# kai0511/insider

Measured on AMD Instinct MI355X. Metric: outer-iterations/sec (masked INSIDER fit, 10000 x 50000, K=30), higher is better.
Workload: dtype f64

## Files before the change

### insider_amd/csrc/insider_hip.hip

```cpp
#include "insider_kernels.hpp"
#include "insider_posthoc.hpp"
#include "insider_vardecomp.hpp"
#include "insider_sampdecomp.hpp"
#include "insider_levelscores.hpp"
#include "insider_factdecomp.hpp"
#include "insider_rescomp.hpp"
#include "insider_outliers.hpp"
#include "insider_neighbors.hpp"
#include "insider_enrich.hpp"
#include "insider_kmeans.hpp"
#include "insider_tsne.hpp"

#include <rccl/rccl.h>

#include <algorithm>
#include <chrono>
#include <cstdlib>
#include <cmath>
#include <cstdio>
#include <cstring>
#include <limits>
#include <memory>
#include <mutex>
#include <atomic>
// ... 227 lines not shown
};

struct Workspace {
    static constexpr int EARLY = 3;
    int K = 0, NB = 0, KP = 0, nseg = 1;
    int gram_blocks_p = 0, gram_blocks_n = 0, sc_blocks = 0;
    DevBuf<double> Astack, R, C, RtR, CCt, Qfull, SC, stat, stat_col, gram_part, sc_part, lvl_part, eq, lvl_sum;
    DevBuf<double> fperm;
    DevBuf<double> lvl_zero;
    DevBuf<double> Qheld;
    DevBuf<double> U, Ylvl, wpart, Vlev;
    DevBuf<double> lvl_sum_all;
    DevBuf<double> gram_part2, sc_part2;
    DevBuf<double> wg_part;
    DevBuf<uint8_t> wg_pair;
    DevBuf<double> sse_train, sse_test, b2, b1, loss_buf, stage;
    size_t stage_count = 0;
    DevBuf<int> sweeps, failflag;
    DevBuf<int> sweep_key;
    DevBuf<unsigned long long> sweep_total;
    DevBuf<unsigned> pc4_ticket;
    unsigned pc4_base[2] = {0, 0};
    unsigned long long cd_code_base = 0, cd_pair_base = 0;
    DevBuf<unsigned long long> code_base_dev;
    uint8_t *order = nullptr;
    DevBuf<uint8_t> order_buf[2];
    int order_rows = 0;
    DevBuf<int> gene_perm;
    DevBuf<int> sched_cnt[2], sched_rank;
    DevBuf<uint16_t> sched_bkt;
    int sched_flip = 0;
    DevBuf<double> cd_hsave, cd_isave;
    DevBuf<uint32_t> cd_pass_slot;
    DevBuf<int> cd_pass_perm[2], cd_pass_cnt;
    DevBuf<int> perm_early[EARLY];
    bool have_early[EARLY] = {false, false, false};
    bool have_perm = false;
};

constexpr unsigned EV_SYNC = hipEventDisableTiming | hipEventDisableSystemFence;

struct Join {
    Event ev;
    bool pending = false;
    int record(hipStream_t s) { HIPCHECK(hipEventRecord(ev, s)); pending = true; return INSIDER_OK; }
    int wait(hipStream_t s)
    {
        if (pending) HIPCHECK(hipStreamWaitEvent(s, ev, 0));
        pending = false;
        return INSIDER_OK;
    }
    void drop() { pending = false; }
};

struct Streams {
    Stream stream;
    Stream side;
    Stream side2;
    Stream side3;
    Event ev_cd_done, ev_prep, ev_c_ready;
    Event ev_head;
    std::vector<Event> ev_w;
    Event ev_a_ready, ev_tab;
    Join qfull, qheld, side_done;

    int create(int n_w)
    {
        HIPCHECK(hipStreamCreate(stream.out()));
        for (Stream *s : {&side, &side2, &side3}) HIPCHECK(hipStreamCreateWithFlags(s->out(), hipStreamNonBlocking));
        for (Event *e : {&ev_prep, &ev_c_ready, &ev_head, &ev_a_ready, &qfull.ev, &qheld.ev, &ev_cd_done, &side_done.ev, &ev_tab})
            HIPCHECK(hipEventCreateWithFlags(e->out(), EV_SYNC));
        ev_w.resize(n_w);
        for (Event &e : ev_w) HIPCHECK(hipEventCreateWithFlags(e.out(), EV_SYNC));
        return INSIDER_OK;
    }
    int synchronize_sides() const
    {
        for (const Stream *s : {&side, &side2, &side3}) HIPCHECK(hipStreamSynchronize(*s));
        return INSIDER_OK;
    }
    void synchronize() const
    {
        for (const Stream *s : {&stream, &side, &side2, &side3}) if (*s) (void)hipStreamSynchronize(*s);
    }
};

struct Options {
    int max_sweeps = 1 << 24, order_mode = 0, profile = 0, verbose = 0, cd_variant = 0, force_allreduce = 0;
    int col_factored = 1;
    int row_counts = 1;
    int row_merged = 1;
    int row_gemm = 1;
    int wg_waves = 1024;
    int row_fused = 1;
    int mm_fast = 1;
    int mm_tiles = 0;
    int col_mfma4 = 1;
    int cd_pairs = 1;
    int list_fine = 1;
    int cd_cold_iters = 3, cd_pass_first = 64, cd_pass_ratio = 4;
    double resid_stage_mb = 256.0;
    double vd_stage_kb = 48.0;
    int sd_slabs = 0;
    int ls_slabs = 0;
    double ls_part_mb = 256.0;
    int glm_slabs = 0;
    int rc_slabs = 0;
};

struct PostWs {
    DevBuf<double> Ast, U, cp, part, stats, stage, gpart, gram, cpart, gsum, L, dinv, outs;
    DevBuf<int> nz, ints, info;
    DevBuf<double> vin, vtab, vrec;
    DevBuf<double> spart, srec;
    DevBuf<double> lcand, ltab, lpart, lcnt, lout;
    DevBuf<double> fwall, fprod, fbase, frec;
    DevBuf<double> rq, rcs, rz, rpart, rin, rout;
    DevBuf<double> ocs, oz;
    DevBuf<uint32_t> obits;
    DevBuf<int> ogcnt, oscnt, orows, ocols;
    DevBuf<long long> ooffs;
};

}

struct insider_hip_handle {
    std::shared_ptr<const DataSet> ds;
    Streams st;
    Options opt;
    Workspace ws;
    PostWs post;
    FitPlan plan;
    bool w_ready = false;
    int64_t gene_offset = 0;
    int rank = 0, world = 1;
    insider_allreduce_fn allreduce = nullptr;
    void *allreduce_user = nullptr;
    ncclComm_t comm = nullptr;
    std::vector<Event> ev_col, ev_row, ev_cd, ev_test;
    double prof[12] = {0, 0, 0, 0, 0, 0, 0, 0, 0, 0, 0, 0};
    double steady_cd_ms = 0, steady_col_ms = 0;
    int cap_hits = 0, max_gene_sweeps = 0;
    int col_solver = 0, col_eval = 0, col_ridge_fallback = 0;
    int col_stats_kernel = 0, col_stats_tickets = 0, col_stats_blocks = 0;
    int col_q_kernel = 0, mm_rows2_tiles = 0;
    uint64_t row_kernels = 0;
    int vd_path = 0;
    int sd_path = 0, sd_slabs = 0;
    int ls_path = 0, ls_slabs = 0;
    int glm_slabs = 0, glm_form = 0;
    int fd_path = 0;
    int rc_slabs = 0;
    double rc_ms = 0.0;
    int ol_path = 0;

    ~insider_hip_handle()
    {
        if (ds) (void)hipSetDevice(ds->device);
        st.synchronize();
        if (comm) (void)ncclCommDestroy(comm);
    }
};

namespace {

constexpr int PC4_PARTS = 16;
constexpr int MM_SLAB = 128;

enum RowKernel {
    RK_WGEMM4 = 0, RK_WGEMM5, RK_WGEMM6, RK_WGEMM7, RK_WGEMM_CHUNKS, RK_WSYRK, RK_GRAM_SIDE,
    RK_GENE_U_CNT, RK_GENE_U, RK_GENE_UC,
    RK_MERGED_SOLVE, RK_MERGED, RK_MERGED_ZERO, RK_PACK_REDUCE,
    RK_LIST_STATS4, RK_LIST_STATS, RK_LEVEL_PARTIAL, RK_LEVEL_SOLVE, RK_CONT_CD,
    RK_MM_ROWS2, RK_MM_ROWS, RK_MM_REDUCE2_2, RK_MM_REDUCE2_4, RK_MM_REDUCE
};
inline uint64_t rk_bit(RowKernel k) { return 1ull << (int)k; }
inline void row_mark(insider_hip_handle *h, RowKernel k) { h->row_kernels |= rk_bit(k); }

PlanFacts plan_facts(const insider_hip_handle *h, int K)
{
    const DataSet &d = *h->ds;
    PlanFacts f;
    const Options &o = h->opt;
    f.opt = {o.row_merged, o.col_factored, o.row_fused, o.row_gemm, o.row_counts, o.mm_fast, o.force_allreduce, o.wg_waves};
    f.world = h->world;
    f.K = K; f.NB = h->ws.NB; f.KP = h->ws.KP; f.lvl_zero = (bool)h->ws.lvl_zero;
    f.merged = d.merged; f.cont_merged = d.cont_merged; f.cf_pair_ok = d.cf_pair_ok; f.cf_hn = (bool)d.cf_hn; f.cf_zt = (bool)d.cf_zt;
    f.c = d.c; f.m = d.m; f.SL = d.SL; f.SLcat = d.SLcat; f.p = d.p; f.col_entries = d.col_entries; f.row_entries = d.row_entries;
    for (const CovTables &ct : d.cov) { f.L.push_back(ct.L); f.npairs.push_back(ct.npairs); }
    f.cf_c = d.cf.c; f.cf_tab_rows = d.cf.tab_rows; f.cf_nsteps = d.cf.nsteps;
    std::copy(d.cf.L, d.cf.L + CF_MAXC + 1, f.cf_L);
    std::copy(d.cf.nlater, d.cf.nlater + CF_MAXC + 1, f.cf_nlater);
    return f;
}

int ensure_workspace(insider_hip_handle *h, int K)
{
    if (K < 1 || K > INSIDER_MAX_K) return fail(INSIDER_ERR_UNSUPPORTED, "K must be in 1..63");
    if (h->ws.K == K) return INSIDER_OK;
    h->ws = Workspace();
    const DataSet &d = *h->ds;
    const hipStream_t st = h->st.stream;
    Workspace w;
    const int NB = (K + 1 + 15) / 16, KP = 16 * NB, NBLK = NB * (NB + 1) / 2, STAT = NBLK * 256;
    w.NB = NB;
    w.KP = KP;
    const int64_t avg_batches = (int64_t)(d.row_entries / (uint64_t)LIST_ALIGN / (uint64_t)std::max<int64_t>(d.n, 1));
    int nseg = (int)std::min<int64_t>(std::max<int64_t>(1, cdiv(8192, d.n)), std::max<int64_t>(1, avg_batches / 16));
    nseg = std::min(nseg, 64);
    w.nseg = nseg;
    w.gram_blocks_p = cdiv(d.p, MM_SLAB);
    w.gram_blocks_n = cdiv(d.n, MM_SLAB);
    w.sc_blocks = cdiv(d.p, MM_SLAB);
    const size_t rec = STAT + 2 * KP + 2, max_L = std::max(d.max_L, 1);
    int rc;
    if ((rc = w.Astack.alloc((size_t)(d.SL + 16) * KP))) return rc;
    HIPCHECK(hipMemset(w.Astack, 0, (size_t)(d.SL + 16) * KP * sizeof(double)));
// ... 35 lines not shown
                }
            if ((rc = w.wg_pair.upload(ab))) return rc;
        }
        if ((rc = w.U.alloc((size_t)d.p * round_up(max_L, 2)))) return rc;
        if ((rc = w.Ylvl.alloc(max_L * KP))) return rc;
        if ((rc = w.wpart.alloc((size_t)std::max(d.max_items, 1) * STAT))) return rc;
        if ((rc = w.lvl_sum_all.alloc((size_t)std::max(d.SL, 1) * rec))) return rc;
        if ((rc = w.gram_part2.alloc((size_t)std::max(w.gram_blocks_p, w.gram_blocks_n) * KP * KP))) return rc;
        if ((rc = w.sc_part2.alloc((size_t)w.sc_blocks * d.SL * KP))) return rc;
        if ((rc = w.Vlev.alloc((size_t)d.p * d.SLP))) return rc;
        HIPCHECK(hipMemsetAsync(w.Vlev, 0, (size_t)d.p * d.SLP * sizeof(double), st));
        if ((rc = w.Qheld.alloc((size_t)d.p * KP))) return rc;
    }
    if ((rc = w.eq.alloc((size_t)d.max_L * (KP * KP + KP)))) return rc;
    for (DevBuf<double> *b : {&w.sse_train, &w.sse_test, &w.b2, &w.b1})
        if ((rc = b->alloc((size_t)d.p))) return rc;
    if ((rc = w.loss_buf.alloc(8))) return rc;
    w.stage_count = (size_t)std::max<int64_t>(std::max<int64_t>(d.p, d.n), d.SL) * KP;
    if ((rc = w.stage.alloc(w.stage_count))) return rc;
    if ((rc = w.sweeps.alloc((size_t)d.p))) return rc;
    if ((rc = w.failflag.alloc(4))) return rc;
    if ((rc = w.sweep_total.alloc(256))) return rc;
    if ((rc = w.pc4_ticket.alloc((size_t)(PC4_PARTS + 1) * 32))) return rc;
    HIPCHECK(hipMemsetAsync(w.pc4_ticket, 0, (size_t)(PC4_PARTS + 1) * 32 * sizeof(unsigned), st));
    if ((rc = w.gene_perm.alloc((size_t)d.p))) return rc;
    if ((rc = w.sched_cnt[0].alloc((size_t)SCHED_BUCKETS))) return rc;
    if ((rc = w.sched_cnt[1].alloc((size_t)SCHED_BUCKETS))) return rc;
    if ((rc = w.sched_rank.alloc((size_t)d.p))) return rc;
    if ((rc = w.sched_bkt.alloc((size_t)d.p))) return rc;
    if ((rc = w.sweep_key.alloc((size_t)d.p))) return rc;
    if ((rc = w.cd_hsave.alloc((size_t)d.p * KP))) return rc;
    if ((rc = w.cd_isave.alloc((size_t)d.p * KP))) return rc;
    if ((rc = w.cd_pass_slot.alloc((size_t)d.p))) return rc;
    if ((rc = w.cd_pass_perm[0].alloc((size_t)d.p))) return rc;
    if ((rc = w.cd_pass_perm[1].alloc((size_t)d.p))) return rc;
    if ((rc = w.cd_pass_cnt.alloc((size_t)CD_BUCKETS + 2))) return rc;
    if ((rc = w.code_base_dev.alloc(2))) return rc;
    for (DevBuf<int> &b : w.perm_early)
        if ((rc = b.alloc((size_t)d.p))) return rc;
    HIPCHECK(hipMemsetAsync(w.sched_cnt[0], 0, SCHED_BUCKETS * sizeof(int), st));
    HIPCHECK(hipMemsetAsync(w.sched_cnt[1], 0, SCHED_BUCKETS * sizeof(int), st));
    HIPCHECK(hipMemsetAsync(w.C, 0, (size_t)(std::max<int64_t>(d.p, d.ldp) + 4) * KP * sizeof(double), st));
    HIPCHECK(hipMemsetAsync(w.R, 0, (size_t)d.n * KP * sizeof(double), st));
    HIPCHECK(hipMemsetAsync(w.failflag, 0, 4 * sizeof(int), st));
    w.K = K;
    h->ws = std::move(w);
    return INSIDER_OK;
}

#define NB_DISPATCH(NBV, ...)                                                           \
    switch (NBV) {                                                                      \
        case 1: { constexpr int NB_ = 1; constexpr int WPB_ = 4; __VA_ARGS__; } break;   \
        case 2: { constexpr int NB_ = 2; constexpr int WPB_ = 4; __VA_ARGS__; } break;   \
        case 3: { constexpr int NB_ = 3; constexpr int WPB_ = 2; __VA_ARGS__; } break;   \
        default: { constexpr int NB_ = 4; constexpr int WPB_ = 1; __VA_ARGS__; } break;  \
    }

#define KT_DISPATCH(KTV, ...)                                   \
    switch (KTV) {                                              \
        case 1: { constexpr int KT_ = 1; __VA_ARGS__; } break;  \
        case 2: { constexpr int KT_ = 2; __VA_ARGS__; } break;  \
        case 3: { constexpr int KT_ = 3; __VA_ARGS__; } break;  \
        default: { constexpr int KT_ = 4; __VA_ARGS__; } break; \
    }

int launch_list_stats(insider_hip_handle *h, bool cols, int nseg, const double *F, double *stat,
                      const double *base = nullptr, uint64_t *mark = nullptr)
{
    const int units = cols ? (int)h->ds->p : (int)h->ds->n;
// ... 191 lines not shown
        HIPCHECK(hipEventRecord(e1, st));
        marked = true;
        return INSIDER_OK;
    }
    int stop_ms(hipStream_t st, float *ms)
    {
        if (!marked)
            if (int rc = mark(st)) return rc;
        HIPCHECK(hipEventSynchronize(e1));
        *ms = 0.0f;
        (void)hipEventElapsedTime(ms, e0, e1);
        return INSIDER_OK;
    }
};

static bool reg3_path(int K, double la) { return K > 32 && K <= 48 && la > 0.0; }

enum ColSolver {
    CS_NONE = 0, CS_RIDGE_REG = 1, CS_RIDGE = 2, CS_CD_REG = 3, CS_CD_REG3 = 4, CS_CD_COLS16 = 5, CS_CD_COLS32 = 6,
    CS_CD_COLS64 = 7, CS_CD_R16_1 = 8, CS_CD_R16_2 = 9, CS_CD_R16_3 = 10
};

static ColSolver cd_solver(int K, double la, int cd_variant)
{
    if (cd_variant == 0 && (K <= 32 || reg3_path(K, la)) && la > 0.0) return K <= 32 ? CS_CD_REG : CS_CD_REG3;
    if (cd_variant == 2 && K <= 16) return CS_CD_R16_1;
    if (cd_variant == 2 && K <= 32) return CS_CD_R16_2;
    if (K <= 16) return CS_CD_COLS16;
    if (K <= 32) return CS_CD_COLS32;
    if (cd_variant != 1 && K <= 48) return CS_CD_R16_3;
    return CS_CD_COLS64;
}

static int launch_cd(ColSolver s, const ColArgs &a, hipStream_t st)
{
    const size_t r16_bytes = (size_t)r16_lds_doubles(a.K) * sizeof(double);
    switch (s) {
        case CS_CD_REG:
        case CS_CD_REG3:
            REG_ANY_DISPATCH(a.K, hipLaunchKernelGGL((k_cd_cols_reg<SL_, KM_, true>), dim3(cdiv(a.p, 4)), dim3(64), 0, st, a));
            break;
        case CS_CD_R16_1: hipLaunchKernelGGL((k_cd_cols_r16<1>), dim3(cdiv(a.p, 4)), dim3(64), r16_bytes, st, a); break;
        case CS_CD_R16_2: hipLaunchKernelGGL((k_cd_cols_r16<2>), dim3(cdiv(a.p, 4)), dim3(64), r16_bytes, st, a); break;
        case CS_CD_R16_3:
            if (int rl = r16_wide_lds(r16_bytes)) return rl;
            hipLaunchKernelGGL((k_cd_cols_r16<3>), dim3(cdiv(a.p, 4)), dim3(64), r16_bytes, st, a);
            break;
        case CS_CD_COLS16: hipLaunchKernelGGL((k_cd_cols<16, 4>), dim3(cdiv(a.p, 16)), dim3(256), 0, st, a); break;
        case CS_CD_COLS32: hipLaunchKernelGGL((k_cd_cols<32, 2>), dim3(cdiv(a.p, 4)), dim3(128), 0, st, a); break;
        case CS_CD_COLS64: hipLaunchKernelGGL((k_cd_cols<64, 1>), dim3((unsigned)a.p), dim3(64), 0, st, a); break;
        default: return fail(INSIDER_ERR_ARG, "not an elastic-net solve kernel");
    }
    KCHECK();
    return INSIDER_OK;
}

static int probe_code_base(int K, unsigned long long *d, hipStream_t st, unsigned long long (&v)[2])
{
    HIPCHECK(hipMemsetAsync(d, 0, 2 * sizeof(unsigned long long), st));
    ColArgs a{};
    a.K = K;
    a.code_base = d;
    REG_DISPATCH(K, hipLaunchKernelGGL((k_cd_cols_reg<SL_, KM_, true>), dim3(1), dim3(64), 0, st, a));
    KCHECK();
    v[0] = v[1] = 0;
    HIPCHECK(hipMemcpyAsync(v, d, sizeof(v), hipMemcpyDeviceToHost, st));
    HIPCHECK(hipStreamSynchronize(st));
    if (!v[0] || !v[1]) return fail(INSIDER_ERR_HIP, "the sweep kernel did not publish the addresses of its code blocks");
    return INSIDER_OK;
}

static int launch_order_table(uint64_t seed, uint32_t iter, int K, int rows, int order_mode, ColSolver s,
                              unsigned long long code_base, unsigned long long pair_base, uint8_t *out, hipStream_t st)
// ... 147 lines not shown

template <typename Args>
void col_args_head(const insider_hip_handle *h, int masked, int checkpoint, Args &a)
{
    a.stat = masked ? h->ws.stat_col : nullptr;
    a.stat_len = h->plan.stat_len;
    a.p = (int)h->ds->p;
    a.K = h->ws.K;
    a.KP = h->ws.KP;
    a.RtR = h->ws.RtR;
    a.Qfull = h->ws.Qfull;
    a.C = h->ws.C;
    a.yy = masked ? h->ds->yy_train : h->ds->yy_all;
    a.checkpoint = checkpoint;
    a.sse_train = h->ws.sse_train;
    a.b2 = h->ws.b2;
    a.b1 = h->ws.b1;
    a.sse_test = h->ws.sse_test;
    a.test_from_stats = masked && h->ds->no_na;
}

int launch_col_solve(insider_hip_handle *h, int masked, bool solve, double lambda, double alpha, double tol,
                     int checkpoint, bool timed, int outer_iter = -1, bool side = false)
{
    const bool early = outer_iter >= 0 && outer_iter < Workspace::EARLY;
    int rc;
    if ((rc = h->st.side_done.wait(h->st.stream))) return rc;
    if ((rc = h->st.qfull.wait(h->st.stream))) return rc;
    Timer t;
    if ((rc = t.begin(h, timed))) return rc;
    bool eval_after = false, fused_bucket = false;
    ColArgs eval_args;
    h->col_solver = h->col_eval = h->col_ridge_fallback = CS_NONE;
    if (alpha == 0.0) {
        RidgeArgs a;
        col_args_head(h, masked, checkpoint, a);
        a.lambda = lambda;
        a.solve = solve ? 1 : 0;
        a.fail = h->ws.failflag;
        a.mark = h->ws.sweeps;
        a.retry = h->ws.failflag + 1;
        a.only_marked = 0;
        if (h->ws.K <= 32 && h->opt.cd_variant == 0) {
            if (solve) {
                HIPCHECK(hipMemsetAsync(h->ws.sweeps, 0, (size_t)h->ds->p * sizeof(int), h->st.stream));
                HIPCHECK(hipMemsetAsync(h->ws.failflag + 1, 0, sizeof(int), h->st.stream));
            }
            REG_DISPATCH(h->ws.K, hipLaunchKernelGGL((k_ridge_cols_reg<SL_, KM_>), dim3(cdiv(h->ds->p, 4)), dim3(64), 0, h->st.stream, a));
            h->col_solver = CS_RIDGE_REG;
            KCHECK();
            if (solve) {
                a.only_marked = 1;
                hipLaunchKernelGGL((k_ridge_cols<1>), dim3((unsigned)h->ds->p), dim3(64), 0, h->st.stream, a);
                h->col_ridge_fallback = 1;
            }
        } else {
            hipLaunchKernelGGL((k_ridge_cols<1>), dim3((unsigned)h->ds->p), dim3(64), 0, h->st.stream, a);
            h->col_solver = CS_RIDGE;
        }
        KCHECK();
        if (solve) HIPCHECK(hipMemsetAsync(h->ws.sweeps, 0, (size_t)h->ds->p * sizeof(int), h->st.stream));
    } else {
        ColArgs a;
        col_args_head(h, masked, checkpoint, a);
        a.mode = solve ? COL_CD : COL_EVAL;
        a.cd.lambda = lambda;
// ... 5 lines not shown
        a.cd.inv_two_la = a.cd.la > 0.0 ? 0.5 / a.cd.la : 0.0;
        a.cd.max_sweeps = h->opt.max_sweeps;
        a.cd.order = h->ws.order;
        a.sweeps = h->ws.sweeps;
        a.sweep_bins = (timed && solve) ? h->ws.sweep_total : nullptr;
        a.gene_perm = !solve ? nullptr : (early && h->ws.have_early[outer_iter]) ? h->ws.perm_early[outer_iter]
                                       : h->ws.have_perm                         ? h->ws.gene_perm
                                                                              : nullptr;
        a.hsave = h->ws.cd_hsave;
        a.isave = h->ws.cd_isave;
        a.pass_count = nullptr;
        a.resume = 0;
        a.pass_slot = nullptr;
        a.bucket_cnt = nullptr;
        a.cap_hits = solve ? h->ws.failflag + 2 : nullptr;
        a.sched_key = a.sched_cnt = a.sched_rank = nullptr;
        a.sched_bkt = nullptr;
        a.sched_reset = 0;
        const ColSolver cs = cd_solver(h->ws.K, a.cd.la, h->opt.cd_variant);
        if (cs == CS_CD_REG || cs == CS_CD_REG3) {
            if (solve) {
                a.sched_key = h->ws.sweep_key;
                a.sched_cnt = h->ws.sched_cnt[h->ws.sched_flip];
                a.sched_rank = h->ws.sched_rank;
                a.sched_bkt = h->ws.sched_bkt;
                a.sched_reset = (outer_iter < Workspace::EARLY || !h->ws.have_perm) ? 1 : 0;
                fused_bucket = true;
            }
            int limits[16], npass = 0;
            if (solve && outer_iter >= 0 && outer_iter < h->opt.cd_cold_iters && h->opt.cd_pass_first >= 32)
                for (int64_t l = h->opt.cd_pass_first; l < std::min<int64_t>(h->opt.max_sweeps, 4 * (int64_t)INSIDER_PERM_PERIOD) && npass < 16;
                     l *= std::max(h->opt.cd_pass_ratio, 2))
                    limits[npass++] = (int)l;
            int start = 0;
            const int *perm_in = a.gene_perm;
            for (int pass = 0;; ++pass) {
                const int limit = pass < npass ? limits[pass] : 0;
                a.cd.start_sweep = start;
                a.cd.sweep_limit = limit;
                a.pass_slot = npass ? h->ws.cd_pass_slot : nullptr;
                a.bucket_cnt = limit ? h->ws.cd_pass_cnt : nullptr;
                if (limit) HIPCHECK(hipMemsetAsync(h->ws.cd_pass_cnt, 0, CD_BUCKETS * sizeof(int), h->st.stream));
                if (solve) {
                    if ((rc = launch_cd(cs, a, h->st.stream))) return rc;
                    h->col_solver = cs;
                }
                if (!limit) break;
                int *count_out = h->ws.cd_pass_cnt + CD_BUCKETS + (pass & 1);
                hipLaunchKernelGGL(k_pass_scatter, dim3(cdiv(h->ds->p, 256)), dim3(256), 0, h->st.stream,
                                   (const uint32_t *)h->ws.cd_pass_slot, (const int *)h->ws.cd_pass_cnt, perm_in, a.pass_count, (int)h->ds->p,
                                   h->ws.cd_pass_perm[pass & 1], count_out);
                KCHECK();
                perm_in = a.gene_perm = h->ws.cd_pass_perm[pass & 1];
                a.pass_count = count_out;
                a.resume = 1;
                start = limit;
            }
            eval_after = checkpoint != 0;
            eval_args = a;
        } else {
            if ((rc = launch_cd(cs, a, h->st.stream))) return rc;
            h->col_solver = cs;
        }
    }
    if ((rc = t.end(h, h->ev_cd))) return rc;
    if (eval_after) {
        eval_args.gene_perm = nullptr;
        eval_args.pass_count = nullptr;
        eval_args.resume = 0;
        if (h->ws.K <= 32) {
            REG_DISPATCH(h->ws.K, hipLaunchKernelGGL((k_cd_cols_reg<SL_, KM_, false>), dim3(cdiv(h->ds->p, 4)), dim3(64), 0, h->st.stream, eval_args));
            h->col_eval = CS_CD_REG;
        } else {
            const size_t eb = (size_t)r16_lds_doubles(h->ws.K) * sizeof(double);
            if (int rl = r16_wide_lds(eb)) return rl;
            eval_args.mode = COL_EVAL;
            hipLaunchKernelGGL((k_cd_cols_r16<3>), dim3(cdiv(h->ds->p, 4)), dim3(64), eb, h->st.stream, eval_args);
            h->col_eval = CS_CD_R16_3;
        }
        KCHECK();
    }
    if (solve && alpha != 0.0) {
        hipStream_t st = h->st.stream;
        if (side) {
            HIPCHECK(hipEventRecord(h->st.ev_cd_done, h->st.stream));
            HIPCHECK(hipStreamWaitEvent(h->st.side, h->st.ev_cd_done, 0));
            st = h->st.side;
        }
        if ((rc = launch_gene_order(h, h->ws.sweeps, (outer_iter < Workspace::EARLY || !h->ws.have_perm) ? 1 : 0, 0, st, fused_bucket)))
            return rc;
// ... 1141 lines not shown
    if (!h || !unique_id || world < 1 || rank < 0 || rank >= world) return fail(INSIDER_ERR_ARG, "bad communicator arguments");
    if (h->world != world || h->rank != rank) return fail(INSIDER_ERR_ARG, "rank / world differ from insider_hip_set_shard()");
    HIPCHECK(hipSetDevice(h->ds->device));
    if (h->comm) { (void)ncclCommDestroy(h->comm); h->comm = nullptr; }
    ncclUniqueId id;
    std::memcpy(&id, unique_id, sizeof(id));
    const ncclResult_t r = ncclCommInitRank(&h->comm, world, id, rank);
    if (r != ncclSuccess) { h->comm = nullptr; return fail(INSIDER_ERR_COMM, std::string("ncclCommInitRank: ") + ncclGetErrorString(r)); }
    return INSIDER_OK;
}

int insider_hip_set_option(insider_hip_handle *h, const char *name, double value)
{
    if (!h || !name) return fail(INSIDER_ERR_ARG, "null");
    const std::string s(name);
    if (s == "max_sweeps") h->opt.max_sweeps = value < 1 ? 1 : (int)value;
    else if (s == "order_mode") h->opt.order_mode = (int)value;
    else if (s == "profile") h->opt.profile = (int)value;
    else if (s == "verbose") h->opt.verbose = (int)value;
    else if (s == "force_allreduce") h->opt.force_allreduce = (int)value;
    else if (s == "col_factored") h->opt.col_factored = (int)value;
    else if (s == "row_counts") h->opt.row_counts = (int)value;
    else if (s == "row_merged") h->opt.row_merged = (int)value;
    else if (s == "row_gemm_waves") {
        h->opt.wg_waves = std::max(64, (int)value);
        HIPCHECK(hipSetDevice(h->ds->device));
        h->ws = Workspace();
    }
    else if (s == "row_gemm") h->opt.row_gemm = (int)value;
    else if (s == "row_fused") h->opt.row_fused = (int)value;
    else if (s == "cd_cold_iters") h->opt.cd_cold_iters = (int)value;
    else if (s == "cd_pass1") h->opt.cd_pass_first = (int)value;
    else if (s == "cd_pass_ratio") h->opt.cd_pass_ratio = (int)value;
    else if (s == "list_fine") h->opt.list_fine = (int)value;
    else if (s == "mm_fast") h->opt.mm_fast = (int)value;
    else if (s == "mm_tiles") h->opt.mm_tiles = value < 1 ? 0 : (int)value;
    else if (s == "col_mfma4") h->opt.col_mfma4 = (int)value;
    else if (s == "cd_pairs") h->opt.cd_pairs = (int)value;
    else if (s == "resid_stage_mb") h->opt.resid_stage_mb = value;
    else if (s == "vd_stage_kb") h->opt.vd_stage_kb = value;
    else if (s == "ls_slabs") h->opt.ls_slabs = value < 1 ? 0 : (int)std::min(value, 256.0);
    else if (s == "rc_slabs") h->opt.rc_slabs = value < 1 ? 0 : (int)std::min(value, 256.0);
    else if (s == "ls_part_mb") h->opt.ls_part_mb = value;
    else if (s == "glm_slabs") h->opt.glm_slabs = value < 1 ? 0 : (int)std::min(value, 64.0);
    else if (s == "sd_slabs") h->opt.sd_slabs = value < 1 ? 0 : (int)std::min(value, 256.0);
    else if (s == "cd_variant") h->opt.cd_variant = (int)value;
    else return fail(INSIDER_ERR_ARG, "unknown option " + s);
    return INSIDER_OK;
}

static void reset_call_state(insider_hip_handle *h, bool drain)
{
    if (drain) (void)hipSetDevice(h->ds->device);
    if (drain) h->st.synchronize();
    h->w_ready = false;
    for (Join *j : {&h->st.qfull, &h->st.qheld, &h->st.side_done}) j->drop();
    clear_events(h);
}

static double decay_for(double delta_loss)
{
    for (double d : {1e-6, 1e-5, 1e-4, 1e-3, 1e-2, 1e-1})
        if (delta_loss / 1000 <= d) return d;
    return 1.0;
}

// ... 1170 lines not shown

double insider_hip_last_cd_ms(void) { return g_last_cd_ms; }
int insider_hip_last_cd_solver(void) { return g_last_cd_solver; }

int insider_hip_get_sweeps(insider_hip_handle *h, int32_t *out)
{
    if (!h || !out) return fail(INSIDER_ERR_ARG, "null");
    if (!h->ws.sweeps) return fail(INSIDER_ERR_ARG, "no column update has run yet");
    HIPCHECK(hipSetDevice(h->ds->device));
    HIPCHECK(hipStreamSynchronize(h->st.stream));
    HIPCHECK(hipMemcpy(out, h->ws.sweeps, (size_t)h->ds->p * sizeof(int), hipMemcpyDeviceToHost));
    return INSIDER_OK;
}

int insider_hip_get_info(insider_hip_handle *h, const char *name, double *out)
{
    if (!h || !name || !out) return fail(INSIDER_ERR_ARG, "null");
    const std::string s(name);
    const int NB = h->ws.NB;
    if (s == "col_stats_path") *out = build_plan(plan_facts(h, h->ws.K), 1).col_path;
    else if (s == "row_merged") *out = build_plan(plan_facts(h, h->ws.K), 1).merged ? 1.0 : 0.0;
    else if (s == "col_entries") *out = (double)h->ds->col_entries;
    else if (s == "row_entries") *out = (double)h->ds->row_entries;
    else if (s == "data_bytes_shared") *out = (double)h->ds->bytes_shared;
    else if (s == "data_bytes_own") *out = (double)h->ds->bytes_own;
    else if (s == "stat_doubles") *out = NB ? NB * (NB + 1) / 2 * 256.0 : 0.0;
    else if (s == "kp") *out = h->ws.KP;
    else if (s == "pair_count_bytes_per_gene") *out = h->ds->cf_pair_ok ? h->ds->cf.cnt_stride : 0.0;
    else if (s == "lists_bytes") *out = 12.0 * ((double)h->ds->col_entries + (double)h->ds->row_entries);
    else if (s == "cap_hits") *out = h->cap_hits;
    else if (s == "max_gene_sweeps") *out = h->max_gene_sweeps;
    else if (s == "max_sweeps") *out = h->opt.max_sweeps;
    else if (s == "col_solver") *out = h->col_solver;
    else if (s == "col_eval") *out = h->col_eval;
    else if (s == "col_ridge_fallback") *out = h->col_ridge_fallback;
    else if (s == "col_stats_kernel") *out = h->col_stats_kernel;
    else if (s == "col_stats_tickets") *out = h->col_stats_tickets;
    else if (s == "col_stats_blocks") *out = h->col_stats_blocks;
    else if (s == "col_q_kernel") *out = h->col_q_kernel;
    else if (s == "mm_rows2_tiles") *out = h->mm_rows2_tiles;
    else if (s == "n_simd") *out = h->ds->n_simd;
    else if (s == "row_kernels") *out = (double)h->row_kernels;
    else if (s == "cd_ms_steady") *out = h->steady_cd_ms;
    else if (s == "col_stats_ms_steady") *out = h->steady_col_ms;
    else if (s == "ol_path") *out = h->ol_path;
    else if (s == "vd_path") *out = h->vd_path;
    else if (s == "sd_path") *out = h->sd_path;
    else if (s == "ls_path") *out = h->ls_path;
    else if (s == "ls_slabs") *out = h->ls_slabs;
    else if (s == "sd_slabs") *out = h->sd_slabs;
    else if (s == "glm_slabs") *out = h->glm_slabs;
    else if (s == "glm_form") *out = h->glm_form;
    else if (s == "rc_slabs") *out = h->rc_slabs;
    else if (s == "rc_ms") *out = h->rc_ms;
    else if (s == "fd_path") *out = h->fd_path;
    else if (s == "col_mfma_per_gene") {
        if (!NB) return fail(INSIDER_ERR_ARG, "no workspace yet: run an update first");
        const int path = build_plan(plan_facts(h, h->ws.K), 1).col_path;
        double v = 0.0;
        if (path == 0) {
            const int NT = (h->ws.K + 4) / 4;
            if (h->opt.list_fine && NB == 2 && NT >= 5 && NT <= 8 && h->ws.fperm)
                v = (double)h->ds->col_entries / (double)std::max<int64_t>(h->ds->p, 1) / 16.0 * (NT * (NT + 1) / 2) / 4.0;
            else
                v = (double)h->ds->col_entries / (double)std::max<int64_t>(h->ds->p, 1) / 4.0 * (NB * (NB + 1) / 2);
        } else
// ... 744 lines not shown
```

### insider_amd/csrc/insider_kernels.hpp

```cpp
#pragma once

#include <hip/hip_runtime.h>
#include <stdint.h>

#include "../../include/insider_perm.h"

namespace insider {

typedef double d4 __attribute__((ext_vector_type(4)));
typedef double d2 __attribute__((ext_vector_type(2)));

constexpr int WAVE = 64;
constexpr int CHUNK = 128;

constexpr int LEVEL_CHUNK = 4;
#define INSIDER_ORDER_ROW 448
constexpr int ORDER_ROW = INSIDER_ORDER_ROW;

constexpr int CODE_TRAIN = 1;
constexpr int CODE_TEST = 2;

template <int NB>
struct Geo {
    static constexpr int KP = 16 * NB;
// ... 724 lines not shown
    int resume;
    uint32_t *pass_slot;
    int *bucket_cnt;
    int *cap_hits;
    int *sched_key, *sched_cnt, *sched_rank;
    uint16_t *sched_bkt;
    int sched_reset;
    unsigned long long *code_base = nullptr;
};

constexpr int CD_BUCKETS = 192;
constexpr uint32_t CD_PASS_DONE = 0xFFFFFFFFu;
__device__ __forceinline__ int cd_bucket(int est) { return CD_BUCKETS - 1 - min(CD_BUCKETS - 1, (int)(8.0f * __log2f((float)max(est, 1)))); }

__global__ void __launch_bounds__(256) k_pass_scatter(const uint32_t *__restrict__ pass_slot, const int *__restrict__ bucket_cnt,
                                                      const int *__restrict__ perm_in, const int *__restrict__ count_in, int p,
                                                      int *__restrict__ perm_out, int *__restrict__ count_out)
{
    __shared__ int off[CD_BUCKETS];
    if (threadIdx.x == 0) {
        int run = 0;
        for (int b = 0; b < CD_BUCKETS; ++b) { off[b] = run; run += bucket_cnt[b]; }
        if (blockIdx.x == 0) *count_out = run;
    }
    __syncthreads();
    const int n_in = count_in ? *count_in : p;
    const int slot = blockIdx.x * 256 + threadIdx.x;
    if (slot >= n_in) return;
    const int j = perm_in ? perm_in[slot] : slot;
    const uint32_t v = pass_slot[j];
    if (v != CD_PASS_DONE) perm_out[off[v >> 24] + (int)(v & 0xFFFFFFu)] = j;
}

template <int W, int WPB>
__global__ void __launch_bounds__(WPB * 64) k_cd_cols(ColArgs a)
{
    constexpr int GPW = 64 / W;
    __shared__ double s_G[WPB][GPW][W * W];
    __shared__ int s_ord[WPB][80];
    const int w = threadIdx.x >> 6, lane = threadIdx.x & 63;
    const int grp = lane / W, l = lane & (W - 1);
    const int slot = (blockIdx.x * WPB + w) * GPW + grp;
    const int j = slot < a.p ? (a.gene_perm ? a.gene_perm[slot] : slot) : a.p;
    const int K = a.K, KP = a.KP;
    const bool gene = j < a.p, valid = gene && l < K;
    double *Goff = s_G[w][grp];
    const double *st = (a.stat && gene) ? a.stat + (size_t)j * a.stat_len : nullptr;
    double Gll = 1.0;
    for (int k = 0; k < K; ++k) {
        double v = 0.0;
        if (valid) {
            v = st ? st[stat_index(k, l)] : a.RtR[k * KP + l];
        }
        if (k == l) { Gll = valid ? v : 1.0; v = 0.0; }
        Goff[k * W + l] = v;
    }
    double q = 0.0, beta = 0.0;
    if (valid) {
        q = a.Qfull[(size_t)j * KP + l];
        if (st) q -= st[stat_index(KP - 1, l)];
        beta = a.C[(size_t)j * KP + l];
    }
    wave_sync();
    double g = 0.0;
    int sweeps = 0;
    if (a.mode == COL_CD) {
// ... 801 lines not shown
```

### insider_amd/csrc/insider_plan.hpp

```cpp
#pragma once

#include <algorithm>
#include <cmath>
#include <cstddef>
#include <cstdint>
#include <vector>

namespace {

inline int64_t round_up(int64_t v, int64_t m) { return (v + m - 1) / m * m; }
inline int cdiv(int64_t a, int64_t b) { return (int)((a + b - 1) / b); }

constexpr int MM_FAST_MIN = 16384;

struct WgPlan {
    bool use = false;
    int tiles = 0, LT = 0, zch = 0, ntile = 0, npair = 0, slab = 0, nslab = 0;
};

struct PlanFacts {
    struct {
        int row_merged, col_factored, row_fused, row_gemm, row_counts, mm_fast, force_allreduce, wg_waves;
    } opt{};
    int world = 1;
    int K = 0, NB = 0, KP = 0;
    bool lvl_zero = false;
    bool merged = false, cont_merged = false, cf_pair_ok = false, cf_hn = false, cf_zt = false;
    int c = 0, m = 0, SL = 0, SLcat = 0;
    int64_t p = 0;
    uint64_t col_entries = 0, row_entries = 0;
    std::vector<int> L;
    std::vector<int64_t> npairs;
    int cf_c = 0, cf_tab_rows = 0, cf_nsteps = 0, cf_L[CF_MAXC + 1] = {0}, cf_nlater[CF_MAXC + 1] = {0};
};

struct FitPlan {
    bool masked = false;
    bool merged = false;
    bool unmasked_fused = false;
    bool fused_solve = false;
    bool mm_fast = false;
    int col_path = 0;
    int NB = 0, KP = 0, stat_len = 0, plen = 0;
    std::vector<WgPlan> wg;
    std::vector<uint8_t> u_cnt;
};

WgPlan wgemm_plan(const PlanFacts &f, int i, bool whatever_the_option = false)
{
    WgPlan w;
    const int K = f.K;
    if (!((f.opt.row_gemm || whatever_the_option) && f.cf_pair_ok && f.cf_hn && f.merged && f.c <= CF_MAXC && K >= 1)) return w;
    const int NB = (K + 1 + 15) / 16;
    const int L = f.L[i], NBLK = NB * (NB + 1) / 2;
    w.tiles = cdiv(L, 16);
    w.npair = K * (K + 1) / 2;
    w.ntile = cdiv(w.npair, 16);
    if (w.tiles < 4 || (double)w.tiles * w.ntile >= 0.9 * (double)L * NBLK) return w;
    w.zch = cdiv(w.tiles, 7);
    w.LT = cdiv(w.tiles, w.zch);
    const int waves_per_slab = cdiv(w.ntile, 2) * w.zch;
    const int want = std::max(1, std::min<int>(f.opt.wg_waves / waves_per_slab, (int)cdiv(f.p, 64)));
    w.slab = (int)round_up(cdiv(f.p, want), 4);
    w.nslab = (int)cdiv(f.p, w.slab);
    w.use = true;
    return w;
}

int col_stats_path(const PlanFacts &f)
{
    if (!(f.merged && f.opt.col_factored && f.c <= CF_MAXC)) return 0;
    if (f.m > 0) return (f.cf_pair_ok && f.cf_zt) ? 2 : 0;
    const bool lookup_fits = ((size_t)(f.cf_tab_rows + 1) * f.KP + 4 * 16 * 17) * sizeof(double) + (size_t)4 * CF_CAP * 2 <= 64 * 1024;
    if (f.opt.col_factored == 3 && f.cf_pair_ok) return 2;
    if (f.opt.col_factored >= 2) return lookup_fits ? 1 : (f.cf_pair_ok ? 2 : 0);
// ... 8 lines not shown
                std::ceil(f.cf_L[t] / 16.0) * ((f.cf_nlater[t] > 0 ? f.cf_nsteps * NB * 64.0 : 0.0) + 150.0);
    }
    double best = list;
    int path = 0;
    if (lookup_fits && 1.3 * fac < best) { best = 1.3 * fac; path = 1; }
    if (f.cf_pair_ok && 1.3 * pair < best) { best = 1.3 * pair; path = 2; }
    return path;
}

bool use_merged(const PlanFacts &f, int masked)
{
    if (!(masked && f.merged && f.opt.row_merged && (f.m == 0 || f.cont_merged))) return false;
    if (f.opt.row_merged == 2 || f.m > 0) return true;
    const int NB = f.NB ? f.NB : 2;
    const double mf = (NB * (NB + 1) / 2) * 16.0 / (1024.0 * 2100.0);
    const double E = (double)f.row_entries, pscale = (double)f.p / 5.0e4;
    const double old_us = E * mf * 1.15 + 50.0 * f.c;
    double merged_us = 0.0;
    for (int i = 0; i < f.c; ++i)
        merged_us += (double)f.npairs[i] * mf * 1.1 + E * (f.c - 1) * 1.3e-6 + 33.0 * pscale * f.SLcat / 110.0 / f.c +
                     37.0 * pscale * f.L[i] / 100.0 + 40.0;
    return 1.1 * merged_us < old_us;
}

FitPlan build_plan(const PlanFacts &f, int masked)
{
    FitPlan p;
    p.masked = masked != 0;
    p.merged = use_merged(f, masked);
    p.unmasked_fused = !masked && f.merged && f.opt.row_merged && f.opt.row_fused && f.m == 0 && f.lvl_zero;
    p.fused_solve = (p.merged || p.unmasked_fused) && f.world <= 1 && !f.opt.force_allreduce && f.opt.row_fused && f.NB <= 2;
    p.mm_fast = f.opt.mm_fast && f.p >= MM_FAST_MIN;
    p.col_path = col_stats_path(f);
    p.NB = f.NB;
    p.KP = f.KP;
    p.stat_len = f.NB * (f.NB + 1) / 2 * 256;
    p.plen = p.stat_len + 2 * f.KP + 2;
    for (int i = 0; i < f.c; ++i) {
        p.wg.push_back(wgemm_plan(f, i));
        const size_t gu_lds = (size_t)4 * (f.SL + round_up(f.L[i], 2) + GU_BATCH * WAVE) * sizeof(double);
        p.u_cnt.push_back(f.cf_pair_ok && (f.opt.row_counts || f.m > 0) && f.c <= CF_MAXC && gu_lds <= 64 * 1024);
    }
    return p;
}

}
```

Baseline: 686.2.

## Split multi-pass column CD solve into two concurrent chains on separate streams

Genes are split into two interleaved halves by quad, each with its own pass-slot permutation and count buffers. The multi-pass coordinate-descent solves then run as two independent chains on the main stream and a new chain stream, with the second chain's pass limits staggered. The aim is to hide the tail and launch gaps between passes, where the remaining active gene set shrinks and the GPU idles, by overlapping the two chains. This adds an extra split kernel, event syncs and more memset/scatter launches, and is enabled only when there are more gene quads than wave slots.

```diff
diff --git a/insider_amd/csrc/insider_hip.hip b/insider_amd/csrc/insider_hip.hip
--- a/insider_amd/csrc/insider_hip.hip
+++ b/insider_amd/csrc/insider_hip.hip
@@ -283,7 +283,10 @@
     int sched_flip = 0;
     DevBuf<double> cd_hsave, cd_isave;
     DevBuf<uint32_t> cd_pass_slot;
-    DevBuf<int> cd_pass_perm[2], cd_pass_cnt;
+    struct PassChain {
+        DevBuf<int> perm[2], cnt;
+        DevBuf<int> order;
+    } cd_chain[2];
     DevBuf<int> perm_early[EARLY];
     bool have_early[EARLY] = {false, false, false};
     bool have_perm = false;
@@ -309,6 +312,8 @@
     Stream side;
     Stream side2;
     Stream side3;
+    Stream chain;
+    Event ev_chain_go, ev_chain_done;
     Event ev_cd_done, ev_prep, ev_c_ready;
     Event ev_head;
     std::vector<Event> ev_w;
@@ -318,8 +323,9 @@
     int create(int n_w)
     {
         HIPCHECK(hipStreamCreate(stream.out()));
-        for (Stream *s : {&side, &side2, &side3}) HIPCHECK(hipStreamCreateWithFlags(s->out(), hipStreamNonBlocking));
-        for (Event *e : {&ev_prep, &ev_c_ready, &ev_head, &ev_a_ready, &qfull.ev, &qheld.ev, &ev_cd_done, &side_done.ev, &ev_tab})
+        for (Stream *s : {&side, &side2, &side3, &chain}) HIPCHECK(hipStreamCreateWithFlags(s->out(), hipStreamNonBlocking));
+        for (Event *e : {&ev_prep, &ev_c_ready, &ev_head, &ev_a_ready, &qfull.ev, &qheld.ev, &ev_cd_done, &side_done.ev, &ev_tab,
+                         &ev_chain_go, &ev_chain_done})
             HIPCHECK(hipEventCreateWithFlags(e->out(), EV_SYNC));
         ev_w.resize(n_w);
         for (Event &e : ev_w) HIPCHECK(hipEventCreateWithFlags(e.out(), EV_SYNC));
@@ -327,12 +333,12 @@
     }
     int synchronize_sides() const
     {
-        for (const Stream *s : {&side, &side2, &side3}) HIPCHECK(hipStreamSynchronize(*s));
+        for (const Stream *s : {&side, &side2, &side3, &chain}) HIPCHECK(hipStreamSynchronize(*s));
         return INSIDER_OK;
     }
     void synchronize() const
     {
-        for (const Stream *s : {&stream, &side, &side2, &side3}) if (*s) (void)hipStreamSynchronize(*s);
+        for (const Stream *s : {&stream, &side, &side2, &side3, &chain}) if (*s) (void)hipStreamSynchronize(*s);
     }
 };
 
@@ -350,6 +356,7 @@
     int cd_pairs = 1;
     int list_fine = 1;
     int cd_cold_iters = 3, cd_pass_first = 64, cd_pass_ratio = 4;
+    int cd_chains = 2, cd_chain_min_waves = -1, cd_chain_stagger = 2;
     double resid_stage_mb = 256.0;
     double vd_stage_kb = 48.0;
     int sd_slabs = 0;
@@ -393,6 +400,7 @@
     double steady_cd_ms = 0, steady_col_ms = 0;
     int cap_hits = 0, max_gene_sweeps = 0;
     int col_solver = 0, col_eval = 0, col_ridge_fallback = 0;
+    int col_chains = 0;
     int col_stats_kernel = 0, col_stats_tickets = 0, col_stats_blocks = 0;
     int col_q_kernel = 0, mm_rows2_tiles = 0;
     uint64_t row_kernels = 0;
@@ -416,6 +424,7 @@
 namespace {
 
 constexpr int PC4_PARTS = 16;
+constexpr int CD_CHAIN_LEN = CD_BUCKETS + 2;
 constexpr int MM_SLAB = 128;
 
 enum RowKernel {
@@ -433,7 +442,9 @@
     const DataSet &d = *h->ds;
     PlanFacts f;
     const Options &o = h->opt;
-    f.opt = {o.row_merged, o.col_factored, o.row_fused, o.row_gemm, o.row_counts, o.mm_fast, o.force_allreduce, o.wg_waves};
+    f.opt = {o.row_merged, o.col_factored, o.row_fused, o.row_gemm, o.row_counts, o.mm_fast, o.force_allreduce, o.wg_waves,
+             o.cd_chains, o.cd_chain_min_waves};
+    f.cd_wave_slots = reg_waves(reg_kmax(K)) * d.n_simd;
     f.world = h->world;
     f.K = K; f.NB = h->ws.NB; f.KP = h->ws.KP; f.lvl_zero = (bool)h->ws.lvl_zero;
     f.merged = d.merged; f.cont_merged = d.cont_merged; f.cf_pair_ok = d.cf_pair_ok; f.cf_hn = (bool)d.cf_hn; f.cf_zt = (bool)d.cf_zt;
@@ -535,9 +546,13 @@
     if ((rc = w.cd_hsave.alloc((size_t)d.p * KP))) return rc;
     if ((rc = w.cd_isave.alloc((size_t)d.p * KP))) return rc;
     if ((rc = w.cd_pass_slot.alloc((size_t)d.p))) return rc;
-    if ((rc = w.cd_pass_perm[0].alloc((size_t)d.p))) return rc;
-    if ((rc = w.cd_pass_perm[1].alloc((size_t)d.p))) return rc;
-    if ((rc = w.cd_pass_cnt.alloc((size_t)CD_BUCKETS + 2))) return rc;
+    for (int c = 0; c < 2; ++c) {
+        const size_t half = (size_t)d.p / 2 + 8;
+        if ((rc = w.cd_chain[c].perm[0].alloc(c ? half : (size_t)d.p))) return rc;
+        if ((rc = w.cd_chain[c].perm[1].alloc(c ? half : (size_t)d.p))) return rc;
+        if ((rc = w.cd_chain[c].cnt.alloc((size_t)CD_BUCKETS + 3))) return rc;
+        if ((rc = w.cd_chain[c].order.alloc(half))) return rc;
+    }
     if ((rc = w.code_base_dev.alloc(2))) return rc;
     for (DevBuf<int> &b : w.perm_early)
         if ((rc = b.alloc((size_t)d.p))) return rc;
@@ -795,13 +810,13 @@
     return CS_CD_COLS64;
 }
 
-static int launch_cd(ColSolver s, const ColArgs &a, hipStream_t st)
+static int launch_cd(ColSolver s, const ColArgs &a, hipStream_t st, int slots = 0)
 {
     const size_t r16_bytes = (size_t)r16_lds_doubles(a.K) * sizeof(double);
     switch (s) {
         case CS_CD_REG:
         case CS_CD_REG3:
-            REG_ANY_DISPATCH(a.K, hipLaunchKernelGGL((k_cd_cols_reg<SL_, KM_, true>), dim3(cdiv(a.p, 4)), dim3(64), 0, st, a));
+            REG_ANY_DISPATCH(a.K, hipLaunchKernelGGL((k_cd_cols_reg<SL_, KM_, true>), dim3(cdiv(slots > 0 ? slots : a.p, 4)), dim3(64), 0, st, a));
             break;
         case CS_CD_R16_1: hipLaunchKernelGGL((k_cd_cols_r16<1>), dim3(cdiv(a.p, 4)), dim3(64), r16_bytes, st, a); break;
         case CS_CD_R16_2: hipLaunchKernelGGL((k_cd_cols_r16<2>), dim3(cdiv(a.p, 4)), dim3(64), r16_bytes, st, a); break;
@@ -1015,6 +1030,7 @@
     bool eval_after = false, fused_bucket = false;
     ColArgs eval_args;
     h->col_solver = h->col_eval = h->col_ridge_fallback = CS_NONE;
+    h->col_chains = 0;
     if (alpha == 0.0) {
         RidgeArgs a;
         col_args_head(h, masked, checkpoint, a);
@@ -1086,30 +1102,71 @@
                 for (int64_t l = h->opt.cd_pass_first; l < std::min<int64_t>(h->opt.max_sweeps, 4 * (int64_t)INSIDER_PERM_PERIOD) && npass < 16;
                      l *= std::max(h->opt.cd_pass_ratio, 2))
                     limits[npass++] = (int)l;
-            int start = 0;
-            const int *perm_in = a.gene_perm;
-            for (int pass = 0;; ++pass) {
-                const int limit = pass < npass ? limits[pass] : 0;
-                a.cd.start_sweep = start;
-                a.cd.sweep_limit = limit;
-                a.pass_slot = npass ? h->ws.cd_pass_slot : nullptr;
-                a.bucket_cnt = limit ? h->ws.cd_pass_cnt : nullptr;
-                if (limit) HIPCHECK(hipMemsetAsync(h->ws.cd_pass_cnt, 0, CD_BUCKETS * sizeof(int), h->st.stream));
-                if (solve) {
-                    if ((rc = launch_cd(cs, a, h->st.stream))) return rc;
-                    h->col_solver = cs;
+            const int p = (int)h->ds->p;
+            const int64_t lim_end = std::min<int64_t>(h->opt.max_sweeps, 4 * (int64_t)INSIDER_PERM_PERIOD);
+            const int nch = (npass > 0 && h->plan.cd_chains && chain_len(p, 1) > 0) ? 2 : 1;
+            struct Chain {
+                ColArgs a;
+                hipStream_t st;
+                Workspace::PassChain *own;
+                const int *perm_in;
+                int slots, start, npass, limits[16];
+            } ch[2];
+            for (int c = 0; c < nch; ++c) {
+                Chain &k = ch[c];
+                k.a = a;
+                k.st = c ? (hipStream_t)h->st.chain : (hipStream_t)h->st.stream;
+                k.own = &h->ws.cd_chain[c];
+                k.perm_in = a.gene_perm;
+                k.slots = k.start = k.npass = 0;
+                for (int i = 0; i < npass; ++i) {
+                    const int64_t l = (int64_t)limits[i] * (c ? h->opt.cd_chain_stagger : 1);
+                    if (l < lim_end) k.limits[k.npass++] = (int)l;
                 }
-                if (!limit) break;
-                int *count_out = h->ws.cd_pass_cnt + CD_BUCKETS + (pass & 1);
-                hipLaunchKernelGGL(k_pass_scatter, dim3(cdiv(h->ds->p, 256)), dim3(256), 0, h->st.stream,
-                                   (const uint32_t *)h->ws.cd_pass_slot, (const int *)h->ws.cd_pass_cnt, perm_in, a.pass_count, (int)h->ds->p,
-                                   h->ws.cd_pass_perm[pass & 1], count_out);
+                if (nch == 2) {
+                    k.perm_in = k.a.gene_perm = k.own->order;
+                    k.a.pass_count = k.own->cnt + CD_CHAIN_LEN;
+                    k.slots = chain_len(p, c);
+                }
+            }
+            if (nch == 2) {
+                hipLaunchKernelGGL(k_chain_split, dim3(cdiv(p, 256)), dim3(256), 0, h->st.stream, a.gene_perm, p,
+                                   (int *)ch[0].own->order, (int *)ch[1].own->order, ch[0].own->cnt + CD_CHAIN_LEN, ch[1].own->cnt + CD_CHAIN_LEN);
                 KCHECK();
-                perm_in = a.gene_perm = h->ws.cd_pass_perm[pass & 1];
-                a.pass_count = count_out;
-                a.resume = 1;
-                start = limit;
+                HIPCHECK(hipEventRecord(h->st.ev_chain_go, h->st.stream));
+                HIPCHECK(hipStreamWaitEvent(h->st.chain, h->st.ev_chain_go, 0));
             }
+            h->col_chains = npass ? nch : 0;
+            for (int pass = 0; pass <= std::max(ch[0].npass, ch[nch - 1].npass); ++pass)
+                for (int c = 0; c < nch; ++c) {
+                    Chain &k = ch[c];
+                    if (pass > k.npass) continue;
+                    const int limit = pass < k.npass ? k.limits[pass] : 0;
+                    k.a.cd.start_sweep = k.start;
+                    k.a.cd.sweep_limit = limit;
+                    k.a.pass_slot = npass ? h->ws.cd_pass_slot : nullptr;
+                    k.a.bucket_cnt = limit ? k.own->cnt : nullptr;
+                    if (limit) HIPCHECK(hipMemsetAsync(k.own->cnt, 0, CD_BUCKETS * sizeof(int), k.st));
+                    if (solve) {
+                        if ((rc = launch_cd(cs, k.a, k.st, k.slots))) return rc;
+                        h->col_solver = cs;
+                    }
+                    if (!limit) continue;
+                    int *count_out = k.own->cnt + CD_BUCKETS + (pass & 1);
+                    hipLaunchKernelGGL(k_pass_scatter, dim3(cdiv(k.slots ? k.slots : p, 256)), dim3(256), 0, k.st,
+                                       (const uint32_t *)h->ws.cd_pass_slot, (const int *)k.own->cnt, k.perm_in, k.a.pass_count, p,
+                                       (int *)k.own->perm[pass & 1], count_out);
+                    KCHECK();
+                    k.perm_in = k.a.gene_perm = k.own->perm[pass & 1];
+                    k.a.pass_count = count_out;
+                    k.a.resume = 1;
+                    k.start = limit;
+                }
+            if (nch == 2) {
+                HIPCHECK(hipEventRecord(h->st.ev_chain_done, h->st.chain));
+                HIPCHECK(hipStreamWaitEvent(h->st.stream, h->st.ev_chain_done, 0));
+            }
+            a = ch[0].a;
             eval_after = checkpoint != 0;
             eval_args = a;
         } else {
@@ -2317,6 +2374,9 @@
     else if (s == "cd_cold_iters") h->opt.cd_cold_iters = (int)value;
     else if (s == "cd_pass1") h->opt.cd_pass_first = (int)value;
     else if (s == "cd_pass_ratio") h->opt.cd_pass_ratio = (int)value;
+    else if (s == "cd_chains") h->opt.cd_chains = value >= 2 ? 2 : 1;
+    else if (s == "cd_chain_min_waves") h->opt.cd_chain_min_waves = value < 0 ? -1 : (int)value;
+    else if (s == "cd_chain_stagger") h->opt.cd_chain_stagger = std::max(1, (int)value);
     else if (s == "list_fine") h->opt.list_fine = (int)value;
     else if (s == "mm_fast") h->opt.mm_fast = (int)value;
     else if (s == "mm_tiles") h->opt.mm_tiles = value < 1 ? 0 : (int)value;
@@ -3553,6 +3613,7 @@
     else if (s == "max_gene_sweeps") *out = h->max_gene_sweeps;
     else if (s == "max_sweeps") *out = h->opt.max_sweeps;
     else if (s == "col_solver") *out = h->col_solver;
+    else if (s == "col_chains") *out = h->col_chains;
     else if (s == "col_eval") *out = h->col_eval;
     else if (s == "col_ridge_fallback") *out = h->col_ridge_fallback;
     else if (s == "col_stats_kernel") *out = h->col_stats_kernel;
diff --git a/insider_amd/csrc/insider_kernels.hpp b/insider_amd/csrc/insider_kernels.hpp
--- a/insider_amd/csrc/insider_kernels.hpp
+++ b/insider_amd/csrc/insider_kernels.hpp
@@ -780,6 +780,21 @@
     if (v != CD_PASS_DONE) perm_out[off[v >> 24] + (int)(v & 0xFFFFFFu)] = j;
 }
 
+__host__ __device__ inline int chain_len(int p, int c)
+{
+    const int nq = (p + 3) / 4, mine = (nq + 1 - c) / 2;
+    return 4 * mine - ((nq > 0 && ((nq - 1) & 1) == c) ? 4 * nq - p : 0);
+}
+__global__ void __launch_bounds__(256) k_chain_split(const int *__restrict__ perm, int p, int *__restrict__ out0, int *__restrict__ out1,
+                                                     int *__restrict__ len0, int *__restrict__ len1)
+{
+    const int s = blockIdx.x * 256 + threadIdx.x;
+    if (s == 0) { *len0 = chain_len(p, 0); *len1 = chain_len(p, 1); }
+    if (s >= p) return;
+    const int w = s >> 2;
+    ((w & 1) ? out1 : out0)[(w >> 1) * 4 + (s & 3)] = perm ? perm[s] : s;
+}
+
 template <int W, int WPB>
 __global__ void __launch_bounds__(WPB * 64) k_cd_cols(ColArgs a)
 {
diff --git a/insider_amd/csrc/insider_plan.hpp b/insider_amd/csrc/insider_plan.hpp
--- a/insider_amd/csrc/insider_plan.hpp
+++ b/insider_amd/csrc/insider_plan.hpp
@@ -21,7 +21,9 @@
 struct PlanFacts {
     struct {
         int row_merged, col_factored, row_fused, row_gemm, row_counts, mm_fast, force_allreduce, wg_waves;
+        int cd_chains, cd_chain_min_waves;
     } opt{};
+    int cd_wave_slots = 0;
     int world = 1;
     int K = 0, NB = 0, KP = 0;
     bool lvl_zero = false;
@@ -41,6 +43,7 @@
     bool fused_solve = false;
     bool mm_fast = false;
     int col_path = 0;
+    bool cd_chains = false;
     int NB = 0, KP = 0, stat_len = 0, plen = 0;
     std::vector<WgPlan> wg;
     std::vector<uint8_t> u_cnt;
@@ -115,6 +118,7 @@
     p.fused_solve = (p.merged || p.unmasked_fused) && f.world <= 1 && !f.opt.force_allreduce && f.opt.row_fused && f.NB <= 2;
     p.mm_fast = f.opt.mm_fast && f.p >= MM_FAST_MIN;
     p.col_path = col_stats_path(f);
+    p.cd_chains = f.opt.cd_chains >= 2 && cdiv(f.p, 4) > (f.opt.cd_chain_min_waves < 0 ? f.cd_wave_slots : f.opt.cd_chain_min_waves);
     p.NB = f.NB;
     p.KP = f.KP;
     p.stat_len = f.NB * (f.NB + 1) / 2 * 256;
```

New measurement: 685.9, median of 3. Within noise of the previous version (-0.0%).
